# david-mathews-1994/deltarice

Hardware: AMD Instinct MI355X
Metric: encode+decode GB/s (int16 in) (higher is better)
Workload: dtype int16; 1 GPU; 1000000x7000 int16 Gaussian(sigma=10), m=8, 500 chunks of 2000x7000 per GPU, encode then decode, HBM resident; waveforms_per_gpu=1000000, wave_len=7000, rice_m=8, chunks_per_gpu=500, decode_impl=8

## Files before the change

### deltarice_amd/csrc/drx_encode.h

```cpp
#ifndef DRX_ENCODE_H
#define DRX_ENCODE_H
#include <hip/hip_runtime.h>
#include <stdint.h>

#include "drx_device.h"

namespace drx {

constexpr int kTile = 512;

typedef uint16_t u16x2 __attribute__((ext_vector_type(2)));
typedef int16_t i16x2 __attribute__((ext_vector_type(2)));
__device__ __forceinline__ u16x2 as_u16x2(uint32_t x) { return __builtin_bit_cast(u16x2, x); }
__device__ __forceinline__ i16x2 as_i16x2(uint32_t x) { return __builtin_bit_cast(i16x2, x); }
__device__ __forceinline__ uint32_t as_u32(u16x2 x) { return __builtin_bit_cast(uint32_t, x); }
__device__ __forceinline__ u16x2 splat(uint32_t v) { return (u16x2){(uint16_t)v, (uint16_t)v}; }

struct PackedCodes { uint32_t nb[4], c16[4], e[4]; };

template <bool GEN>
__device__ __forceinline__ void packed_codes(const uint32_t x[4], uint32_t xprev, uint32_t xprev2, const u16x2 (&tp)[4],
                                             uint32_t k, PackedCodes &c) {
    const u16x2 kv = splat(k), kp1 = splat(k + 1u), c16k = splat(16u - k);
    const u16x2 mlo = splat((1u << k) - 1u), mdelta = splat(0xffffu - ((1u << k) - 1u));
    u16x2 z[4], qc[4], e[4];
#pragma unroll
    for (int j = 0; j < 4; ++j) {
        const uint32_t xm1 = j ? x[j - 1] : xprev;
        const uint32_t before = __builtin_amdgcn_alignbit(x[j], xm1, 16);
        i16x2 d;
        if (GEN) {
            const uint32_t xm2 = j >= 2 ? x[j - 2] : (j == 1 ? xprev : xprev2);
            const uint32_t before3 = __builtin_amdgcn_alignbit(xm1, xm2, 16);
            d = __builtin_bit_cast(i16x2, (u16x2)(as_u16x2(x[j]) * tp[0] + as_u16x2(before) * tp[1] +
                                                  as_u16x2(xm1) * tp[2] + as_u16x2(before3) * tp[3]));
        } else {
            d = as_i16x2(x[j]) - as_i16x2(before);
        }
        z[j] = __builtin_bit_cast(u16x2, (i16x2)(d << (int16_t)1)) ^
               __builtin_bit_cast(u16x2, (i16x2)(d >> (int16_t)15));
    }
#pragma unroll
    for (int j = 0; j < 4; ++j) qc[j] = __builtin_elementwise_min((u16x2)(z[j] >> kv), splat(8u));
#pragma unroll
    for (int j = 0; j < 4; ++j) e[j] = qc[j] >> (uint16_t)3;
#pragma unroll
    for (int j = 0; j < 4; ++j) c.nb[j] = as_u32(e[j] * c16k + (qc[j] + kp1));
    const uint32_t mword = as_u32(splat(1u << k));
#pragma unroll
    for (int j = 0; j < 4; ++j) {
        const uint32_t mask = as_u32(e[j] * mdelta + mlo);
        c.c16[j] = (mask & as_u32(z[j])) | (~mask & mword);
        c.e[j] = as_u32(e[j]);
    }
}

constexpr uint32_t kEncCapWords = 2048;

__device__ __forceinline__ int load8_dwords(const int16_t *__restrict__ x, uint32_t len, uint32_t t0, int lane,
                                            bool vec_ok, uint32_t w[4]) {
    const uint32_t i0 = t0 + 8u * (uint32_t)lane;
    const int nv = (i0 >= len) ? 0 : (int)((len - i0) < 8u ? (len - i0) : 8u);
    if (vec_ok && nv == 8) {
        const uint4 q = *reinterpret_cast<const uint4 *>(x + i0);
        w[0] = q.x; w[1] = q.y; w[2] = q.z; w[3] = q.w;
    } else {
#pragma unroll
        for (int j = 0; j < 4; ++j) {
            const uint32_t a = (2 * j < nv) ? (uint32_t)(uint16_t)x[i0 + 2 * j] : 0u;
            const uint32_t b = (2 * j + 1 < nv) ? (uint32_t)(uint16_t)x[i0 + 2 * j + 1] : 0u;
            w[j] = a | (b << 16);
        }
    }
    return nv;
}

__device__ __forceinline__ void mask_tail(PackedCodes &c, int nv) {
#pragma unroll
    for (int j = 0; j < 4; ++j) {
        const uint32_t m = (2 * j + 1 < nv) ? 0xffffffffu : ((2 * j < nv) ? 0x0000ffffu : 0u);
        c.nb[j] &= m;
    }
}

__device__ __forceinline__ uint32_t lane_tile_bits(const PackedCodes &c) {
    const u16x2 s = as_u16x2(c.nb[0]) + as_u16x2(c.nb[1]) + as_u16x2(c.nb[2]) + as_u16x2(c.nb[3]);
    const uint32_t v = as_u32(s);
    return (v & 0xffffu) + (v >> 16);
}

template <bool FULL>
__device__ __forceinline__ void emit_tile(const PackedCodes &c, uint32_t pb) {
    typedef uint32_t __attribute__((address_space(3))) lds_u32;
#pragma unroll
    for (int j = 0; j < 8; ++j) {
        const uint32_t n = (j & 1) ? (c.nb[j >> 1] >> 16) : (c.nb[j >> 1] & 0xffffu);
        uint32_t code32 = __builtin_amdgcn_perm(c.e[j >> 1], c.c16[j >> 1], (j & 1) ? 0x07060302u : 0x05040100u);
        if (!FULL) code32 = n ? code32 : 0u;
        const uint32_t pe = pb + n;
        const uint64_t v = (uint64_t)code32 << (((pb & 32u) - pe) & 63u);
        lds_u32 *w = (lds_u32 *)(uintptr_t)((pb >> 3) & ~3u);
        __hip_atomic_fetch_or(w, (uint32_t)(v >> 32), __ATOMIC_RELAXED, __HIP_MEMORY_SCOPE_WORKGROUP);
        if ((uint32_t)v) __hip_atomic_fetch_or(w + 1, (uint32_t)v, __ATOMIC_RELAXED, __HIP_MEMORY_SCOPE_WORKGROUP);
        pb = pe;
    }
}

__device__ __forceinline__ void concat_codes(const PackedCodes &c, uint32_t (&w)[4]) {
    uint32_t w0 = 0, w1 = 0, w2 = 0, w3 = 0;
#pragma unroll
    for (int j = 0; j < 8; ++j) {
        const uint32_t nbj = c.nb[j >> 1];
        const uint32_t n = (j & 1) ? (nbj >> 16) : nbj;
        const uint32_t code32 = __builtin_amdgcn_perm(c.e[j >> 1], c.c16[j >> 1], (j & 1) ? 0x07060302u : 0x05040100u);
        const uint32_t s = 0u - n;
        if (j >= 3) w3 = __builtin_amdgcn_alignbit(w3, w2, s);
        if (j >= 2) w2 = __builtin_amdgcn_alignbit(w2, w1, s);
        if (j >= 1) w1 = __builtin_amdgcn_alignbit(w1, w0, s);
        w0 = (w0 << (n & 31u)) | code32;
    }
    w[0] = w0; w[1] = w1; w[2] = w2; w[3] = w3;
}

__device__ __forceinline__ void place_words(const uint32_t (&wd)[4], uint32_t pe) {
    typedef uint32_t __attribute__((address_space(3))) lds_u32;
    const uint32_t x0 = __builtin_amdgcn_alignbit(wd[0], 0u, pe);
    const uint32_t x1 = __builtin_amdgcn_alignbit(wd[1], wd[0], pe);
    const uint32_t x2 = __builtin_amdgcn_alignbit(wd[2], wd[1], pe);
    const uint32_t x3 = __builtin_amdgcn_alignbit(wd[3], wd[2], pe);
    const uint32_t x4 = __builtin_amdgcn_alignbit(0u, wd[3], pe);
    lds_u32 *w = (lds_u32 *)(uintptr_t)(((pe >> 3) & ~3u) - 16u);
    __hip_atomic_fetch_or(w + 4, x0, __ATOMIC_RELAXED, __HIP_MEMORY_SCOPE_WORKGROUP);
    __hip_atomic_fetch_or(w + 3, x1, __ATOMIC_RELAXED, __HIP_MEMORY_SCOPE_WORKGROUP);
    __hip_atomic_fetch_or(w + 2, x2, __ATOMIC_RELAXED, __HIP_MEMORY_SCOPE_WORKGROUP);
    if (x3 | x4) {
        __hip_atomic_fetch_or(w + 1, x3, __ATOMIC_RELAXED, __HIP_MEMORY_SCOPE_WORKGROUP);
        if (x4) __hip_atomic_fetch_or(w, x4, __ATOMIC_RELAXED, __HIP_MEMORY_SCOPE_WORKGROUP);
    }
}

constexpr uint32_t kBufFront = 4;

__device__ __forceinline__ void zero_row(uint32_t *row, uint32_t words, int lane) {
    for (int i = lane; i < (int)(words / 4u); i += 64) reinterpret_cast<uint4 *>(row)[i] = make_uint4(0, 0, 0, 0);
}

struct TileCodes {
    PackedCodes c;
    uint32_t cw[4], lane_bits, incl, tile_bits;
};

template <bool GEN, bool FULLT>
__device__ __forceinline__ TileCodes code_tile(const uint32_t (&w)[4], int nv, uint32_t &carry, uint32_t &carry2, const u16x2 (&tp)[4],
                                               uint32_t k) {
    TileCodes t;
    const uint32_t xprev = wave_shr1_carry(w[3], carry);
    carry = (uint32_t)__builtin_amdgcn_readlane((int)w[3], 63);
    uint32_t xprev2 = 0;
    if (GEN) {
        xprev2 = wave_shr1_carry(w[2], carry2);
        carry2 = (uint32_t)__builtin_amdgcn_readlane((int)w[2], 63);
    }
    packed_codes<GEN>(w, xprev, xprev2, tp, k, t.c);
    if (!FULLT) mask_tail(t.c, nv);
    t.lane_bits = lane_tile_bits(t.c);
    if (FULLT) concat_codes(t.c, t.cw);
    t.incl = wave_incl_scan_dpp(t.lane_bits);
    t.tile_bits = (uint32_t)__builtin_amdgcn_readlane((int)t.incl, 63);
    return t;
}

template <bool FULLT, typename At>
__device__ __forceinline__ void put_tile(const TileCodes &t, At &&at) {
    if (FULLT && !__any(t.lane_bits > 128u))
        place_words(t.cw, at(t.incl));
    else
        emit_tile<FULLT>(t.c, at(t.incl - t.lane_bits));
}

__device__ __forceinline__ void shr128(uint32_t (&w)[4], uint32_t n) {
    const uint32_t ws = n >> 5;
    const uint32_t y0 = ws == 0u ? w[0] : ws == 1u ? w[1] : ws == 2u ? w[2] : ws == 3u ? w[3] : 0u;
    const uint32_t y1 = ws == 0u ? w[1] : ws == 1u ? w[2] : ws == 2u ? w[3] : 0u;
    const uint32_t y2 = ws == 0u ? w[2] : ws == 1u ? w[3] : 0u;
    const uint32_t y3 = ws == 0u ? w[3] : 0u;
    w[0] = __builtin_amdgcn_alignbit(y1, y0, n);
    w[1] = __builtin_amdgcn_alignbit(y2, y1, n);
    w[2] = __builtin_amdgcn_alignbit(y3, y2, n);
    w[3] = y3 >> (n & 31u);
}

template <bool GEN>
__device__ __forceinline__ TileCodes code_tail_tile(const uint32_t (&w)[4], int nv, bool ragged, uint32_t &carry, uint32_t &carry2,
                                                    const u16x2 (&tp)[4], uint32_t k, bool &wide) {
    TileCodes t;
    const uint32_t xprev = wave_shr1_carry(w[3], carry);
    carry = (uint32_t)__builtin_amdgcn_readlane((int)w[3], 63);
    uint32_t xprev2 = 0;
    if (GEN) {
        xprev2 = wave_shr1_carry(w[2], carry2);
        carry2 = (uint32_t)__builtin_amdgcn_readlane((int)w[2], 63);
    }
    packed_codes<GEN>(w, xprev, xprev2, tp, k, t.c);
    const uint32_t all_bits = lane_tile_bits(t.c);
    concat_codes(t.c, t.cw);
    if (ragged) {
        PackedCodes cm = t.c;
        mask_tail(cm, nv);
        t.lane_bits = lane_tile_bits(cm);
        shr128(t.cw, all_bits - t.lane_bits);
    } else {
        t.lane_bits = nv ? all_bits : 0u;
#pragma unroll
        for (int j = 0; j < 4; ++j) t.cw[j] = nv ? t.cw[j] : 0u;
    }
    wide = __any((nv ? all_bits : 0u) > 128u);
    t.incl = wave_incl_scan_dpp(t.lane_bits);
    t.tile_bits = (uint32_t)__builtin_amdgcn_readlane((int)t.incl, 63);
    return t;
}

template <typename At>
__device__ __forceinline__ void put_tail_tile(const TileCodes &t, int nv, bool wide, At &&at) {
    if (!wide) {
        place_words(t.cw, at(t.incl));
    } else {
        PackedCodes c = t.c;
        mask_tail(c, nv);
        emit_tile<false>(c, at(t.incl - t.lane_bits));
    }
}

template <typename B, typename F>
__device__ __forceinline__ void for_full_tiles(const int16_t *__restrict__ x, uint32_t n_full, int lane, B &&between, F &&full) {
    constexpr int kDepth = 3;
    const uint4 *xv = reinterpret_cast<const uint4 *>(x) + lane;
    uint4 q[kDepth];
    uint32_t t = 0;
#pragma unroll
    for (int u = 0; u < kDepth; ++u) {
        q[u] = make_uint4(0, 0, 0, 0);
        if ((uint32_t)u < n_full) q[u] = xv[64 * (size_t)u];
    }
#pragma unroll 1
    for (; t + 2u * kDepth <= n_full; t += kDepth) {
        between();
#pragma unroll
        for (int u = 0; u < kDepth; ++u) {
            const uint32_t w[4] = {q[u].x, q[u].y, q[u].z, q[u].w};
            full(w);
            q[u] = xv[64 * (size_t)(t + u + kDepth)];
        }
    }
#pragma unroll 1
    for (; t < n_full; t += kDepth) {
        between();
#pragma unroll
        for (int u = 0; u < kDepth; ++u) {
            if (t + (uint32_t)u < n_full) {
                const uint32_t w[4] = {q[u].x, q[u].y, q[u].z, q[u].w};
                full(w);
                if (t + (uint32_t)u + kDepth < n_full) q[u] = xv[64 * (size_t)(t + u + kDepth)];
            }
        }
    }
}

template <typename B, typename F, typename T>
__device__ __forceinline__ void for_tiles(const int16_t *__restrict__ x, uint32_t len, uint32_t n_full, bool tail, int lane,
                                          B &&between, F &&full, T &&tailf) {
    constexpr int kDepth = 3;
    const uint32_t last = tail ? n_full : n_full - 1u;
    const uint32_t imax = len - 8u;
    auto load = [&](uint32_t tile) -> uint4 {
        tile = tile < last ? tile : last;
        uint32_t i = tile * (uint32_t)kTile + 8u * (uint32_t)lane;
        i = i < imax ? i : imax;
        return *reinterpret_cast<const uint4 *>(x + i);
    };
    uint4 q[kDepth];
#pragma unroll
    for (int u = 0; u < kDepth; ++u) {
        q[u] = load((uint32_t)u);
        __builtin_amdgcn_sched_barrier(0);
    }
    uint32_t t = 0;
#pragma unroll 1
    for (; t + kDepth <= n_full; t += kDepth) {
        between(true);
#pragma unroll
        for (int u = 0; u < kDepth; ++u) {
            const uint32_t w[4] = {q[u].x, q[u].y, q[u].z, q[u].w};
            full(w);
            q[u] = load(t + (uint32_t)u + kDepth);
        }
    }
    const uint32_t left = n_full - t;
    static_assert(kDepth == 3, "the straight code below");
    if (left) {
        between(false);
        const uint32_t w0[4] = {q[0].x, q[0].y, q[0].z, q[0].w};
        full(w0);
        if (left > 1u) {
            const uint32_t w1[4] = {q[1].x, q[1].y, q[1].z, q[1].w};
            full(w1);
        }
    }
    if (tail) {
        auto sel = [left](uint32_t a, uint32_t b, uint32_t c) -> uint32_t { return left == 0u ? a : (left == 1u ? b : c); };
        const uint32_t w[4] = {sel(q[0].x, q[1].x, q[2].x), sel(q[0].y, q[1].y, q[2].y), sel(q[0].z, q[1].z, q[2].z),
                               sel(q[0].w, q[1].w, q[2].w)};
        tailf(w);
    } else {
        __builtin_amdgcn_s_waitcnt(0x0f70);
    }
}

template <bool GEN, bool WINDOW>
__device__ __forceinline__ uint64_t recode_tiles(const int16_t *__restrict__ x, uint32_t len, uint32_t carry, uint32_t carry2,
                                                 const u16x2 (&tp)[4], uint32_t k, int lane, uint32_t *row, uint32_t row_words,
                                                 uint32_t *__restrict__ outp, uint32_t P0, uint32_t skip, uint32_t limit, uint64_t cap) {
    zero_row(row, row_words, lane);
    wave_sync();
    uint32_t *buf = row + kBufFront;
    const uint32_t buf_bits = lds_addr(buf) * 8u;
    auto mine = [&](uint64_t idx) -> bool { return !WINDOW || (idx >= skip && idx < limit && idx < cap); };
    uint64_t P = P0;
    uint32_t wn[4];
    int nvn = load8_dwords(x, len, 0u, lane, true, wn);
    for (uint32_t t0 = 0; t0 < len; t0 += kTile) {
        const uint32_t w[4] = {wn[0], wn[1], wn[2], wn[3]};
        const int nv = nvn;
        if (t0 + kTile < len) nvn = load8_dwords(x, len, t0 + kTile, lane, true, wn);
        const TileCodes t = code_tile<GEN, false>(w, nv, carry, carry2, tp, k);
        const uint64_t wfirst = P >> 5;
        const uint32_t at0 = buf_bits + (uint32_t)(P & 31u);
        put_tile<false>(t, [&](uint32_t bit) -> uint32_t { return at0 + bit; });
        P += t.tile_bits;
        wave_sync();
        const uint32_t nfull = (uint32_t)((P >> 5) - wfirst);
        for (uint32_t i = lane; i < nfull; i += 64) {
            if (mine(wfirst + i)) outp[wfirst + i] = buf[i];
            buf[i] = 0;
        }
        wave_sync();
        if (nfull && lane == 0) { const uint32_t cwd = buf[nfull]; buf[nfull] = 0; buf[0] = cwd; }
        wave_sync();
    }
    if (lane == 0) {
        if ((P & 31u) && mine(P >> 5)) outp[P >> 5] = buf[0];
        buf[0] = 0;
    }
    wave_sync();
    return P;
}

template <bool GEN>
__device__ __forceinline__ uint64_t recode_waveform(const int16_t *__restrict__ x, uint32_t len, const u16x2 (&tp)[4], uint32_t k, int lane,
                                                    uint32_t *row, uint32_t row_words, uint32_t *__restrict__ outp) {
    return recode_tiles<GEN, false>(x, len, 0u, 0u, tp, k, lane, row, row_words, outp, 0u, 0u, 0u, 0ull);
}

template <bool GEN>
__device__ __forceinline__ void history_before(const int16_t *__restrict__ x, uint32_t &carry, uint32_t &carry2) {
    carry = (uint32_t)(uint16_t)x[-1] << 16;
    if (GEN) {
        carry |= (uint32_t)(uint16_t)x[-2];
        carry2 = (uint32_t)(uint16_t)x[-4] | ((uint32_t)(uint16_t)x[-3] << 16);
    }
}

template <bool GEN>
__device__ __forceinline__ void recode_range(const int16_t *__restrict__ xw, uint32_t wf_len, uint32_t s_begin, uint32_t s_end, uint64_t Bp,
                                             uint32_t bits_mine, const u16x2 (&tp)[4], uint32_t k, int lane, uint32_t *row,
                                             uint32_t row_words, uint32_t *__restrict__ payload, uint64_t cap_words) {
    const uint32_t P0 = (uint32_t)(Bp & 31u);
    const uint64_t wbase = Bp >> 5;
    const uint32_t more = wf_len - s_end < 32u ? wf_len - s_end : 32u;
    uint32_t carry = 0, carry2 = 0;
    if (s_begin) history_before<GEN>(xw + s_begin, carry, carry2);
    recode_tiles<GEN, true>(xw + s_begin, s_end - s_begin + more, carry, carry2, tp, k, lane, row, row_words, payload + wbase, P0,
                            P0 ? 1u : 0u, (P0 + bits_mine + 31u) >> 5, cap_words > wbase ? cap_words - wbase : 0ull);
}

}
#endif
```

### deltarice_amd/csrc/drx_encode_stream.hip

```cpp
#include <hip/hip_runtime.h>
#include <stdint.h>

#include <type_traits>

#include "drx_internal.h"
#include "drx_device.h"
#include "drx_encode.h"

namespace drx {

constexpr int kEsWaves = 4;
constexpr uint32_t kEsFront = kBufFront;
constexpr uint32_t kEsBack = 12;
constexpr uint64_t kEsFlag = 1ull << 63;
constexpr uint32_t kEsCtrlWords = 32;
constexpr uint32_t kEsRing = kEsRingWords;
constexpr int kEsPollSleep = 4;

__device__ __forceinline__ uint64_t es_load(const uint64_t *p) {
    return __hip_atomic_load(p, __ATOMIC_RELAXED, __HIP_MEMORY_SCOPE_AGENT);
}
__device__ __forceinline__ void es_store(uint64_t *p, uint64_t v) {
    __hip_atomic_store(p, v, __ATOMIC_RELAXED, __HIP_MEMORY_SCOPE_AGENT);
}

constexpr uint32_t kScPer = 8;

__device__ __forceinline__ void es_scanner(uint64_t total, const uint64_t *__restrict__ size, uint64_t *__restrict__ place,
                                           DevStatus *st) {
    const int lane = lane_id();
    if (threadIdx.x >= 64) return;
    __builtin_amdgcn_s_setprio(3);
    uint64_t pos = 0, base = 0;
    uint32_t idle = 0;
    auto sample = [&](uint64_t (&v)[kScPer], uint64_t at) {
#pragma unroll
        for (int j = 0; j < (int)kScPer; ++j) {
            const uint64_t e = at + 64u * j + (uint32_t)lane;
            v[j] = e < total ? es_load(size + e) : kEsFlag;
        }
    };
    while (pos < total) {
        uint64_t v[kScPer];
        const uint64_t bs = pos;
        sample(v, pos);
        uint64_t run = 0;
        bool open = true, big = false;
#pragma unroll
        for (int j = 0; j < (int)kScPer; ++j) {
            const uint64_t e = bs + 64u * j + (uint32_t)lane;
            const uint64_t m = __ballot(e < pos || (v[j] >> 63) != 0);
            const uint32_t l = (m == ~0ull) ? 64u : (uint32_t)__builtin_ctzll(~m);
            run += open ? l : 0u;
            open = open && l == 64u;
            big = big || __any((v[j] & ~kEsFlag) >= (1ull << 24));
        }
        uint64_t end = bs + run;
        end = end < total ? end : total;
        if (end <= pos) {
            if (++idle > (1u << 22)) {
                if (lane == 0) atomicOr(&st->err, kErrInternal);
                return;
            }
            __builtin_amdgcn_s_sleep(1);
            continue;
        }
        idle = 0;
        uint64_t running = 0;
#pragma unroll
        for (int j = 0; j < (int)kScPer; ++j) {
            if (bs + 64u * j < end) {
                const uint64_t e = bs + 64u * j + (uint32_t)lane;
                const bool in = e >= pos && e < end;
                const uint64_t val = in ? (v[j] & ~kEsFlag) : 0ull;
                uint64_t inc;
                if (!big) {
                    inc = wave_incl_scan_dpp((uint32_t)val);
                } else {
                    inc = val;
#pragma unroll
                    for (int d = 1; d < 64; d <<= 1) {
                        const uint64_t t = __shfl_up(inc, d);
                        if (lane >= d) inc += t;
                    }
                }
                if (in) es_store(place + e, kEsFlag | (base + running + inc - val));
                running += big ? __shfl(inc, 63) : (uint64_t)(uint32_t)__builtin_amdgcn_readlane((int)(uint32_t)inc, 63);
            }
        }
        base += running;
        pos = end;
    }
}

template <int WV>
struct EsShared {
    uint32_t role, arrive, ticket[4];
    uint64_t mine[2][WV];
    uint32_t place_t[2];
};

template <int WV>
__device__ __forceinline__ uint32_t es_rendezvous(EsShared<WV> &shm, uint32_t cyc, int lane, int wv, uint32_t *__restrict__ ctrl,
                                                  uint64_t *__restrict__ size, uint32_t Tprev, uint64_t &off) {
    typedef uint32_t __attribute__((address_space(3))) lds_u32;
    uint32_t arr = 0;
    if (lane == 0) arr = __hip_atomic_fetch_add((lds_u32 *)&shm.arrive, 1u, __ATOMIC_RELAXED, __HIP_MEMORY_SCOPE_WORKGROUP);
    arr = (uint32_t)__builtin_amdgcn_readfirstlane((int)arr);
    if (arr == (uint32_t)WV * cyc) {
        if (lane == 0) shm.ticket[cyc & 3u] = atomicAdd(ctrl + 32, 1u);
    }
    __syncthreads();
    const uint32_t T = rfl(shm.ticket[cyc & 3u]);
    if (cyc) {
        uint64_t sum = 0, before = 0;
#pragma unroll
        for (int i = 0; i < WV; ++i) {
            const uint64_t m = rfl64(shm.mine[(cyc - 1u) & 1u][i]);
            sum += m;
            before += i < wv ? m : 0ull;
        }
        off = before;
        if (wv == 0 && lane == 0) es_store(size + Tprev, kEsFlag | sum);
    }
    return T;
}

template <uint32_t RING>
__device__ __forceinline__ uint32_t es_gap(bool pend, uint32_t startA, uint32_t start, uint32_t behind) {
    if (!pend) return RING - 8u;
    const uint32_t d = startA >= start ? startA - start : startA + RING - start;
    return d > behind ? d - behind : 0u;
}

template <typename InLds, typename Wait, typename Copy>
__device__ __forceinline__ bool es_release(bool must, uint64_t P, InLds &&place_in_lds, Wait &&wait_place, Copy &&copy_out) {
    decltype(wait_place()) pl;
    const bool seen = place_in_lds(pl);
    if (!(seen || must)) return false;
    if (!seen) __builtin_amdgcn_s_setprio(0);
    else if (P < (uint64_t)(4u * kTile * 7u)) __builtin_amdgcn_s_setprio(2);
    else __builtin_amdgcn_s_setprio(1);
    copy_out(seen ? pl : wait_place());
    return true;
}

template <uint32_t RING, typename Put>
__device__ __forceinline__ void ring_put_with(const TileCodes &t, uint32_t *row, uint32_t s0, int lane, Put &&put) {
    constexpr uint32_t kRingBits = RING * 32u;
    uint32_t *ring = row + kEsFront;
    const uint32_t ring_bits0 = lds_addr(ring) * 8u;
    put([&](uint32_t bit) -> uint32_t {
        const uint32_t b = s0 + bit;
        return ring_bits0 + (b >= kRingBits ? b - kRingBits : b);
    });
    if (s0 < kRingBits && s0 + t.tile_bits >= kRingBits) {
        wave_sync();
        if (lane < (int)kEsFront) {
            const uint32_t v = row[lane];
            if (v) { ring[RING - kEsFront + lane] |= v; row[lane] = 0; }
        } else if (lane < (int)(kEsFront + kEsBack)) {
            const uint32_t i = (uint32_t)lane - kEsFront, v = ring[RING + i];
            if (v) { ring[i] |= v; ring[RING + i] = 0; }
        }
        wave_sync();
    }
}
template <bool FULLT, uint32_t RING>
__device__ __forceinline__ void ring_put(const TileCodes &t, uint32_t *row, uint32_t s0, int lane) {
    ring_put_with<RING>(t, row, s0, lane, [&](auto &&at) { put_tile<FULLT>(t, at); });
}

static unsigned es_grid(const Geom &G, uint64_t tickets) {
    const unsigned full = 256u * (16u / kEsWaves);
    return (G.dbg & DRX_DBG_STREAM_THREE_WGS) ? 3u : (unsigned)(tickets + 1 < full ? tickets + 1 : full);
}

template <bool GEN, int WV, uint32_t RING>
__global__ __launch_bounds__(64 * WV, 4) void k_encode_stream(Geom G, const int16_t *__restrict__ in, uint32_t *__restrict__ out,
                                                              uint64_t out_cap, uint64_t *__restrict__ chunk_word_off,
                                                              uint32_t *__restrict__ wave_words, uint64_t *__restrict__ size,
                                                              uint64_t *__restrict__ place, uint32_t *__restrict__ ctrl,
                                                              DevStatus *st) {
    __shared__ __attribute__((aligned(16))) uint32_t ring_all[WV][kEsFront + RING + kEsBack];
    __shared__ EsShared<WV> shm;
    __shared__ uint64_t s_place_v[2];
    typedef uint32_t __attribute__((address_space(3))) lds_u32;
    typedef uint64_t __attribute__((address_space(3))) lds_u64;
    static_assert((kEsFront + RING + kEsBack) % 4 == 0 && RING % 4 == 0, "16-byte LDS accesses");
    constexpr uint32_t kRowWords = kEsFront + RING + kEsBack;
    const int lane = lane_id(), wv = wave_id();
    uint32_t *row = ring_all[wv];
    uint32_t *ring = row + kEsFront;

    if (threadIdx.x == 0) {
        shm.role = atomicAdd(ctrl, 1u);
        shm.arrive = 0;
        shm.place_t[0] = shm.place_t[1] = 0;
    }
    zero_row(row, kRowWords, lane);
    __syncthreads();
    const uint64_t n_tickets = (G.total_waves + WV - 1) / WV;
    if (rfl(shm.role) == 0) {
        es_scanner(n_tickets, size, place, st);
        return;
    }

    const uint32_t k = G.k;
    const u16x2 tp[4] = {splat(GEN ? G.enc_t[0] : 1u), splat(GEN ? G.enc_t[1] : 0xffffu), splat(GEN ? G.enc_t[2] : 0u),
                         splat(GEN ? G.enc_t[3] : 0u)};

    bool pend = false, fitsA = true;
    uint64_t gA = 0, offA = 0;
    uint32_t TA = 0, startA = 0, nA = 0;
    WaveRef rA = {};

    auto place_header = [&](const WaveRef &r, uint64_t g, uint32_t n, uint64_t ex, uint64_t &pos) -> bool {
        const uint64_t mine = 1ull + n + (r.idx == 0 ? 1ull : 0ull);
        pos = ex + (r.idx == 0 ? 1ull : 0ull);
        if (lane == 0) {
            if (r.idx == 0) chunk_word_off[r.chunk] = ex;
            if (g + 1 == G.total_waves) {
                chunk_word_off[G.n_chunks] = ex + mine;
                st->total_words = ex + mine;
                if (G.host_words) *G.host_words = ex + mine;
                if (ex + mine > out_cap) atomicOr(&st->err, kErrCapacity);
            }
        }
        const bool room = pos + 1u + n <= out_cap;
        if (room && lane == 0) {
            out[pos] = n;
            if (r.idx == 0) out[pos - 1] = r.n_samples;
        }
        return room;
    };
    auto copy_out = [&](uint64_t ex) {
        uint64_t pos;
        const bool room = place_header(rA, gA, nA, ex + offA, pos);
        uint32_t *__restrict__ outp = out + pos + 1;
        typedef uint32_t u32x4s __attribute__((ext_vector_type(4)));
        typedef u32x4s __attribute__((address_space(1), aligned(4))) g_u32x4_a4;
        const uint32_t n4 = nA & ~3u;
        for (uint32_t i = 4u * (uint32_t)lane; i < n4; i += 256u) {
            uint32_t w = startA + i;
            w = w >= RING ? w - RING : w;
            const uint4 v = *reinterpret_cast<const uint4 *>(ring + w);
            if (room) *(g_u32x4_a4 *)(outp + i) = (u32x4s){v.x, v.y, v.z, v.w};
            *reinterpret_cast<uint4 *>(ring + w) = make_uint4(0, 0, 0, 0);
        }
        if ((uint32_t)lane < nA - n4) {
            uint32_t w = startA + n4 + (uint32_t)lane;
            w = w >= RING ? w - RING : w;
            if (room) outp[n4 + (uint32_t)lane] = ring[w];
            ring[w] = 0;
        }
        wave_sync();
        pend = false;
    };
    auto place_in_lds = [&](uint64_t &ex) -> bool {
        const uint32_t t = __hip_atomic_load((lds_u32 *)&shm.place_t[TA & 1u], __ATOMIC_RELAXED, __HIP_MEMORY_SCOPE_WORKGROUP);
        if (rfl(t) != TA + 1u) return false;
        ex = rfl64(__hip_atomic_load((lds_u64 *)&s_place_v[TA & 1u], __ATOMIC_RELAXED, __HIP_MEMORY_SCOPE_WORKGROUP));
        return true;
    };
    auto place_to_lds = [&](uint64_t ex) {
        if (lane == 0) {
            __hip_atomic_store((lds_u64 *)&s_place_v[TA & 1u], ex, __ATOMIC_RELAXED, __HIP_MEMORY_SCOPE_WORKGROUP);
            __hip_atomic_store((lds_u32 *)&shm.place_t[TA & 1u], TA + 1u, __ATOMIC_RELAXED, __HIP_MEMORY_SCOPE_WORKGROUP);
        }
    };
    auto wait_place = [&]() -> uint64_t {
        uint32_t spins = 0;
        for (;;) {
            uint64_t ex;
            bool have = place_in_lds(ex);
            if (!have) {
                uint64_t v = 0;
                if (lane == 0) v = es_load(place + TA);
                const uint32_t hi = (uint32_t)__builtin_amdgcn_readfirstlane((int)(uint32_t)(v >> 32));
                if (hi >> 31) {
                    ex = ((uint64_t)(hi & 0x7fffffffu) << 32) | (uint32_t)__builtin_amdgcn_readfirstlane((int)(uint32_t)v);
                    place_to_lds(ex);
                    have = true;
                }
            }
            if (have) return ex;
            __builtin_amdgcn_s_sleep(kEsPollSleep);
            if (++spins > (1u << 22)) {
                if (lane == 0) atomicOr(&st->err, kErrInternal);
                return out_cap;
            }
        }
    };

    auto stream_out = [&](uint64_t ex) {
        uint64_t pos;
        const bool room = place_header(rA, gA, nA, ex + offA, pos);
        recode_waveform<GEN>(in + rA.sample_off, room ? rA.len : 0u, tp, k, lane, row, kRowWords, out + pos + 1);
        pend = false;
    };

    uint32_t start = 0;
    uint32_t Tprev = 0;
    for (uint32_t cyc = 0;; ++cyc) {
        const uint32_t T = es_rendezvous(shm, cyc, lane, wv, ctrl, size, Tprev, offA);
        if (pend && !fitsA) stream_out(wait_place());
        if ((uint64_t)T * WV >= G.total_waves) break;
        Tprev = T;
        const uint64_t g = (uint64_t)T * WV + (uint32_t)wv;
        if (g >= G.total_waves) {
            if (lane == 0) shm.mine[cyc & 1u][wv] = 0;
            if (pend) copy_out(wait_place());
            continue;
        }

        const WaveRef r = locate_uniform(G, g);
        const int16_t *x = in + r.sample_off;
        const uint32_t wlen = r.len;
        const uint32_t n_full = wlen / kTile, rem = wlen - n_full * (uint32_t)kTile;
        const bool tail = rem != 0u, ragged = (rem & 7u) != 0u;
        const bool tail_lane = 8u * (uint32_t)lane + 8u <= rem;

        auto gap = [&]() -> uint32_t { return es_gap<RING>(pend, startA, start, 8u); };
        if (pend && gap() < 512u) copy_out(wait_place());
        uint32_t limit = gap();

        uint64_t P = 0;
        bool fits = true;
        uint32_t carry = 0;
        uint32_t carry2 = 0;
        auto process_tile = [&](const uint32_t (&w)[4], int nv, auto full_tag) {
            constexpr bool FULLT = decltype(full_tag)::value;
            bool wide = false;
            TileCodes t;
            if constexpr (FULLT) t = code_tile<GEN, true>(w, nv, carry, carry2, tp, k);
            else t = code_tail_tile<GEN>(w, nv, ragged, carry, carry2, tp, k, wide);
            const uint32_t need = ((uint32_t)P + t.tile_bits + 31u) >> 5;
            bool ok = fits && need < limit;
            if (pend && es_release(fits && !ok, P, place_in_lds, wait_place, copy_out)) {
                limit = gap();
                ok = fits && need < limit;
            }
            if (ok) {
                if constexpr (FULLT) ring_put<true, RING>(t, row, start * 32u + (uint32_t)P, lane);
                else ring_put_with<RING>(t, row, start * 32u + (uint32_t)P, lane, [&](auto &&at) { put_tail_tile(t, nv, wide, at); });
            } else {
                fits = false;
            }
            P += t.tile_bits;
        };
        uint64_t pollv = 0;
        bool polling = false;
        auto between = [&](bool again) {
            if (!pend) return;
            if (polling) {
                const uint32_t hi = (uint32_t)__builtin_amdgcn_readfirstlane((int)(uint32_t)(pollv >> 32));
                polling = false;
                if (hi >> 31) {
                    place_to_lds(((uint64_t)(hi & 0x7fffffffu) << 32) | (uint32_t)__builtin_amdgcn_readfirstlane((int)(uint32_t)pollv));
                    return;
                }
            }
            if (!again) return;
            if (lane == 0) pollv = es_load(place + TA);
            polling = true;
        };

        auto full_tile = [&](const uint32_t (&w)[4]) { process_tile(w, 8, std::true_type{}); };
        auto tail_tile = [&](const uint32_t (&wq)[4]) {
            const uint32_t i0 = 8u * (uint32_t)lane;
            const int nv = tail_lane ? 8 : (i0 < rem ? (int)(rem - i0) : 0);
            uint32_t w[4];
#pragma unroll
            for (int j = 0; j < 4; ++j) w[j] = tail_lane ? wq[j] : 0u;
            if (ragged && nv > 0 && nv < 8) {
                const int16_t *xl = x + (size_t)n_full * kTile + i0;
#pragma unroll
                for (int j = 0; j < 4; ++j) {
                    const uint32_t a = (2 * j < nv) ? (uint32_t)(uint16_t)xl[2 * j] : 0u;
                    const uint32_t b = (2 * j + 1 < nv) ? (uint32_t)(uint16_t)xl[2 * j + 1] : 0u;
                    w[j] = a | (b << 16);
                }
            }
            process_tile(w, nv, std::false_type{});
        };
        if (wlen >= 8u) {
            for_tiles(x, wlen, n_full, tail, lane, between, full_tile, tail_tile);
        } else {
            const uint32_t none[4] = {0u, 0u, 0u, 0u};
            tail_tile(none);
        }
        const uint32_t n = (uint32_t)((P + 31u) >> 5);
        wave_sync();
        if (lane == 0) {
            wave_words[g] = n;
            shm.mine[cyc & 1u][wv] = 1ull + n + (r.idx == 0 ? 1ull : 0ull);
        }
        if (pend) copy_out(wait_place());
        pend = true;
        fitsA = fits;
        gA = g;
        rA = r;
        TA = T;
        startA = start;
        nA = n;
        if (fits) {
            start += (n + 3u) & ~3u;
            start = start >= RING ? start - RING : start;
        }
    }
    if (pend) copy_out(wait_place());
}

struct EsPlace2 { uint64_t whdr, bits; };

__device__ __forceinline__ void es_scanner_segs(uint64_t total, uint32_t tpw, uint32_t waves_per_chunk, const uint64_t *__restrict__ size,
                                                uint64_t *__restrict__ place, DevStatus *st) {
    const int lane = lane_id();
    if (threadIdx.x >= 64) return;
    __builtin_amdgcn_s_setprio(3);
    uint64_t pos = 0;
    uint64_t whdr = 1;
    uint64_t bits_in = 0;
    uint32_t idle = 0;
    const double rcp_tpw = 1.0 / (double)tpw;
    while (pos < total) {
        uint64_t v[kScPer];
        const uint64_t bs = pos;
#pragma unroll
        for (int j = 0; j < (int)kScPer; ++j) {
            const uint64_t e = bs + 64u * j + (uint32_t)lane;
            v[j] = e < total ? es_load(size + e) : 0ull;
        }
        uint64_t run = 0;
        bool open = true;
#pragma unroll
        for (int j = 0; j < (int)kScPer; ++j) {
            const uint64_t m = __ballot((v[j] >> 63) != 0);
            const uint32_t l = (m == ~0ull) ? 64u : (uint32_t)__builtin_ctzll(~m);
            run += open ? l : 0u;
            open = open && l == 64u;
        }
        const uint64_t end = bs + run;
        if (end <= pos) {
            if (++idle > (1u << 22)) {
                if (lane == 0) atomicOr(&st->err, kErrInternal);
                return;
            }
            __builtin_amdgcn_s_sleep(1);
            continue;
        }
        idle = 0;
#pragma unroll
        for (int j = 0; j < (int)kScPer; ++j) {
            if (bs + 64u * j < end) {
                const uint64_t e = bs + 64u * j + (uint32_t)lane;
                const bool in = e < end;
                const uint32_t val = in ? (uint32_t)(v[j] & 0xffffffffull) : 0u;
                const uint32_t e32 = (uint32_t)e;
                uint32_t g = (uint32_t)((double)e32 * rcp_tpw);
                uint32_t jj = e32 - g * tpw;
                if ((int32_t)jj < 0) { g -= 1u; jj += tpw; }
                if (jj >= tpw) { g += 1u; jj -= tpw; }
                const bool closing = in && jj + 1u == tpw;
                const uint32_t inc = wave_incl_scan_dpp(val), ex = inc - val;
                const int f = lane - (int)jj;
                const uint32_t exf = (uint32_t)__shfl((int)ex, f < 0 ? 0 : f);
                const uint64_t before = f < 0 ? bits_in + ex : (uint64_t)(ex - exf);
                const uint64_t nw = closing ? (before + val + 31ull) >> 5 : 0ull;
                const uint64_t contrib = closing ? 1ull + nw + (((g + 1u) % waves_per_chunk == 0u) ? 1ull : 0ull) : 0ull;
                uint64_t cinc;
                if (!__any(contrib >= (1ull << 24))) {
                    cinc = wave_incl_scan_dpp((uint32_t)contrib);
                } else {
                    cinc = contrib;
#pragma unroll
                    for (int d = 1; d < 64; d <<= 1) {
                        const uint64_t t = __shfl_up(cinc, d);
                        if (lane >= d) cinc += t;
                    }
                }
                const uint64_t my_whdr = whdr + cinc - contrib;
                if (in) {
                    es_store(place + 2u * e, kEsFlag | my_whdr);
                    es_store(place + 2u * e + 1u, kEsFlag | before);
                }
                const uint64_t left = end - (bs + 64u * j);
                const int li = __builtin_amdgcn_readfirstlane(left >= 64u ? 63 : (int)left - 1);
                const uint64_t wn = my_whdr + contrib, bn = closing ? 0ull : before + val;
                whdr = ((uint64_t)(uint32_t)__builtin_amdgcn_readlane((int)(uint32_t)(wn >> 32), li) << 32) | (uint32_t)__builtin_amdgcn_readlane((int)(uint32_t)wn, li);
                bits_in = ((uint64_t)(uint32_t)__builtin_amdgcn_readlane((int)(uint32_t)(bn >> 32), li) << 32) | (uint32_t)__builtin_amdgcn_readlane((int)(uint32_t)bn, li);
            }
        }
        pos = end;
    }
}

template <bool GEN, int WV, uint32_t RING>
__global__ __launch_bounds__(64 * WV, 4) void k_encode_stream_segs(Geom G, uint32_t seg_len, uint32_t tpw, const int16_t *__restrict__ in,
                                                                   uint32_t *__restrict__ out, uint64_t out_cap,
                                                                   uint64_t *__restrict__ chunk_word_off, uint32_t *__restrict__ wave_words,
                                                                   uint64_t *__restrict__ size, uint64_t *__restrict__ place,
                                                                   uint32_t *__restrict__ ctrl, DevStatus *st) {
    __shared__ __attribute__((aligned(16))) uint32_t ring_all[WV][kEsFront + RING + kEsBack];
    __shared__ EsShared<WV> shm;
    __shared__ uint64_t s_place_v[2][2];
    __shared__ uint32_t s_first[2][WV];
    typedef uint32_t __attribute__((address_space(3))) lds_u32;
    typedef uint64_t __attribute__((address_space(3))) lds_u64;
    static_assert((kEsFront + RING + kEsBack) % 4 == 0 && RING % 4 == 0, "16-byte LDS accesses");
    static_assert(WV == (int)kEsSegWaves, "es_seg_shape() counts tickets of kEsSegWaves segments");
    constexpr uint32_t kRowWords = kEsFront + RING + kEsBack;
    const int lane = lane_id(), wv = wave_id();
    uint32_t *row = ring_all[wv];
    uint32_t *ring = row + kEsFront;

    if (threadIdx.x == 0) {
        shm.role = atomicAdd(ctrl, 1u);
        shm.arrive = 0;
        shm.place_t[0] = shm.place_t[1] = 0;
    }
    zero_row(row, kRowWords, lane);
    __syncthreads();
    const uint64_t n_tickets = G.total_waves * tpw;
    if (rfl(shm.role) == 0) {
        es_scanner_segs(n_tickets, tpw, G.u_n_waves, size, place, st);
        return;
    }
    const uint32_t k = G.k;
    const u16x2 tp[4] = {splat(GEN ? G.enc_t[0] : 1u), splat(GEN ? G.enc_t[1] : 0xffffu), splat(GEN ? G.enc_t[2] : 0u),
                         splat(GEN ? G.enc_t[3] : 0u)};

    bool pend = false, fitsA = true, lastA = false, sibA = false;
    uint64_t gA = 0, offA = 0;
    uint32_t TA = 0, startA = 0, nA = 0, bitsA = 0, sbeginA = 0, sendA = 0, parA = 0;
    WaveRef rA = {};

    auto headers = [&](const WaveRef &r, const EsPlace2 &pl, uint64_t B) {
        if (lane != 0) return;
        if (sbeginA == 0u && r.idx == 0u) {
            chunk_word_off[r.chunk] = pl.whdr - 1u;
            if (pl.whdr - 1u < out_cap) out[pl.whdr - 1u] = r.n_samples;
        }
        if (lastA) {
            const uint64_t n = (B + bitsA + 31ull) >> 5;
            wave_words[gA] = (uint32_t)n;
            if (pl.whdr < out_cap) out[pl.whdr] = (uint32_t)n;
            if (gA + 1u == G.total_waves) {
                const uint64_t tot = pl.whdr + 1ull + n;
                chunk_word_off[G.n_chunks] = tot;
                st->total_words = tot;
                if (G.host_words) *G.host_words = tot;
                if (tot > out_cap) atomicOr(&st->err, kErrCapacity);
            }
        }
    };
    auto copy_out = [&](const EsPlace2 &pl) {
        const uint64_t B = pl.bits + offA;
        headers(rA, pl, B);
        const uint64_t w0 = pl.whdr + 1ull + (B >> 5);
        const uint32_t s = (uint32_t)B & 31u;
        const uint32_t i_lo = s ? 1u : 0u, i_hi = (s + bitsA + 31u) >> 5;
        const uint32_t nA4 = (nA + 3u) & ~3u, top = nA4 > i_hi ? nA4 : ((i_hi + 3u) & ~3u);
        if (sibA) {
            if (lane == 0) {
                const uint32_t F = s_first[parA][wv + 1], sh = bitsA & 31u;
                uint32_t wi = startA + (bitsA >> 5);
                wi = wi >= RING ? wi - RING : wi;
                ring[wi] |= F >> sh;
                if (sh) {
                    wi = wi + 1u >= RING ? wi + 1u - RING : wi + 1u;
                    ring[wi] |= F << (32u - sh);
                }
            }
            wave_sync();
        }
        uint32_t *__restrict__ outp = out + w0;
        const uint64_t room = out_cap > w0 ? out_cap - w0 : 0ull;
        typedef uint32_t u32x4s __attribute__((ext_vector_type(4)));
        typedef u32x4s __attribute__((address_space(1), aligned(4))) g_u32x4_a4;
        uint32_t carryw = 0;
        for (uint32_t i0 = 0; i0 < top; i0 += 256u) {
            const uint32_t i = i0 + 4u * (uint32_t)lane;
            uint4 v = make_uint4(0, 0, 0, 0);
            uint32_t w = startA + i;
            w = w >= RING ? w - RING : w;
            const bool inr = i < nA4;
            if (inr) v = *reinterpret_cast<const uint4 *>(ring + w);
            uint32_t pw = (uint32_t)__builtin_amdgcn_update_dpp(0, (int)v.w, 0x138, 0xf, 0xf, false);
            if (lane == 0) pw = carryw;
            carryw = (uint32_t)__builtin_amdgcn_readlane((int)v.w, 63);
            const uint32_t o0 = __builtin_amdgcn_alignbit(pw, v.x, s), o1 = __builtin_amdgcn_alignbit(v.x, v.y, s);
            const uint32_t o2 = __builtin_amdgcn_alignbit(v.y, v.z, s), o3 = __builtin_amdgcn_alignbit(v.z, v.w, s);
            if (i >= i_lo && i + 4u <= i_hi && (uint64_t)i + 4u <= room) {
                *(g_u32x4_a4 *)(outp + i) = (u32x4s){o0, o1, o2, o3};
            } else {
                if (i >= i_lo && i < i_hi && (uint64_t)i < room) outp[i] = o0;
                if (i + 1u >= i_lo && i + 1u < i_hi && (uint64_t)i + 1u < room) outp[i + 1u] = o1;
                if (i + 2u >= i_lo && i + 2u < i_hi && (uint64_t)i + 2u < room) outp[i + 2u] = o2;
                if (i + 3u >= i_lo && i + 3u < i_hi && (uint64_t)i + 3u < room) outp[i + 3u] = o3;
            }
            if (inr) *reinterpret_cast<uint4 *>(ring + w) = make_uint4(0, 0, 0, 0);
        }
        wave_sync();
        pend = false;
    };
    auto place_in_lds = [&](EsPlace2 &pl) -> bool {
        const uint32_t t = __hip_atomic_load((lds_u32 *)&shm.place_t[TA & 1u], __ATOMIC_RELAXED, __HIP_MEMORY_SCOPE_WORKGROUP);
        if (rfl(t) != TA + 1u) return false;
        pl.whdr = rfl64(__hip_atomic_load((lds_u64 *)&s_place_v[TA & 1u][0], __ATOMIC_RELAXED, __HIP_MEMORY_SCOPE_WORKGROUP));
        pl.bits = rfl64(__hip_atomic_load((lds_u64 *)&s_place_v[TA & 1u][1], __ATOMIC_RELAXED, __HIP_MEMORY_SCOPE_WORKGROUP));
        return true;
    };
    auto place_to_lds = [&](const EsPlace2 &pl) {
        if (lane == 0) {
            __hip_atomic_store((lds_u64 *)&s_place_v[TA & 1u][0], pl.whdr, __ATOMIC_RELAXED, __HIP_MEMORY_SCOPE_WORKGROUP);
            __hip_atomic_store((lds_u64 *)&s_place_v[TA & 1u][1], pl.bits, __ATOMIC_RELAXED, __HIP_MEMORY_SCOPE_WORKGROUP);
            __hip_atomic_store((lds_u32 *)&shm.place_t[TA & 1u], TA + 1u, __ATOMIC_RELAXED, __HIP_MEMORY_SCOPE_WORKGROUP);
        }
    };
    auto place_of = [&](uint64_t pv, EsPlace2 &pl) -> bool {
        const uint32_t lo = (uint32_t)pv, hi = (uint32_t)(pv >> 32);
        const uint32_t h0 = (uint32_t)__builtin_amdgcn_readlane((int)hi, 0), h1 = (uint32_t)__builtin_amdgcn_readlane((int)hi, 1);
        if (!((h0 & h1) >> 31)) return false;
        pl.whdr = ((uint64_t)(h0 & 0x7fffffffu) << 32) | (uint32_t)__builtin_amdgcn_readlane((int)lo, 0);
        pl.bits = ((uint64_t)(h1 & 0x7fffffffu) << 32) | (uint32_t)__builtin_amdgcn_readlane((int)lo, 1);
        return true;
    };
    auto wait_place = [&]() -> EsPlace2 {
        uint32_t spins = 0;
        for (;;) {
            EsPlace2 pl;
            if (place_in_lds(pl)) return pl;
            uint64_t pv = 0;
            if (lane < 2) pv = es_load(place + 2ull * TA + (uint32_t)lane);
            if (place_of(pv, pl)) {
                place_to_lds(pl);
                return pl;
            }
            __builtin_amdgcn_s_sleep(kEsPollSleep);
            if (++spins > (1u << 22)) {
                if (lane == 0) atomicOr(&st->err, kErrInternal);
                pl.whdr = out_cap;
                pl.bits = 0;
                return pl;
            }
        }
    };

    auto stream_out = [&](const EsPlace2 &pl) {
        const uint64_t B = pl.bits + offA;
        headers(rA, pl, B);
        recode_range<GEN>(in + rA.sample_off, rA.len, sbeginA, sendA, B, bitsA, tp, k, lane, row, kRowWords, out + pl.whdr + 1ull,
                          out_cap > pl.whdr + 1ull ? out_cap - pl.whdr - 1ull : 0ull);
        pend = false;
    };

    uint32_t start = 0;
    uint32_t Tprev = 0;
    for (uint32_t cyc = 0;; ++cyc) {
        const uint32_t T = es_rendezvous(shm, cyc, lane, wv, ctrl, size, Tprev, offA);
        if (pend && !fitsA) stream_out(wait_place());
        if ((uint64_t)T >= n_tickets) break;
        Tprev = T;
        const uint32_t gw = T / tpw, tj = T - gw * tpw;
        const uint64_t g = gw;
        const WaveRef r = locate_uniform(G, g);
        const uint32_t wlen = r.len;
        const uint32_t sgi = tj * (uint32_t)WV + (uint32_t)wv;
        const uint64_t sb64 = (uint64_t)sgi * seg_len;
        if (sb64 >= wlen) {
            if (lane == 0) shm.mine[cyc & 1u][wv] = 0;
            if (pend) copy_out(wait_place());
            continue;
        }
        const uint32_t s_begin = (uint32_t)sb64;
        const uint32_t s_end = wlen - s_begin > seg_len ? s_begin + seg_len : wlen;
        const bool sib = wv + 1 < WV && seg_len >= 32u && wlen - s_end >= 32u;
        const uint32_t more = sib ? 0u : (wlen - s_end < 32u ? wlen - s_end : 32u);
        const uint32_t slen = s_end - s_begin;
        const uint32_t clen = slen + more;
        const int16_t *x = in + r.sample_off + s_begin;

        auto gap = [&]() -> uint32_t { return es_gap<RING>(pend, startA, start, 12u); };
        if (pend && gap() < 512u) copy_out(wait_place());
        uint32_t limit = gap();

        uint64_t P = 0;
        uint32_t seg_bits = 0;
        bool first = true;
        bool fits = true;
        uint32_t carry = 0, carry2 = 0;
        if (s_begin) history_before<GEN>(x, carry, carry2);
        auto process_tile = [&](const uint32_t (&w)[4], int nv, int mark, auto full_tag) {
            constexpr bool FULLT = decltype(full_tag)::value;
            const TileCodes t = code_tile<GEN, FULLT>(w, nv, carry, carry2, tp, k);
            if (!FULLT && mark >= 0) seg_bits = (uint32_t)P + (mark ? (uint32_t)__builtin_amdgcn_readlane((int)t.incl, mark - 1) : 0u);
            const uint32_t need = ((uint32_t)P + t.tile_bits + 31u) >> 5;
            bool ok = fits && need < limit;
            if (pend && es_release(fits && !ok, P, place_in_lds, wait_place, copy_out)) {
                limit = gap();
                ok = fits && need < limit;
            }
            if (ok)
                ring_put<FULLT, RING>(t, row, start * 32u + (uint32_t)P, lane);
            else
                fits = false;
            P += t.tile_bits;
            if (first) {
                first = false;
                wave_sync();
                if (lane == 0) s_first[cyc & 1u][wv] = ring[start];
            }
        };
        const uint32_t n_fast = more ? slen / kTile : clen / kTile;
        uint64_t pollv = 0;
        bool polling = false;
        auto between = [&]() {
            if (!pend) return;
            if (polling) {
                polling = false;
                EsPlace2 pl;
                if (place_of(pollv, pl)) {
                    place_to_lds(pl);
                    return;
                }
            }
            pollv = 0;
            if (lane < 2) pollv = es_load(place + 2ull * TA + (uint32_t)lane);
            polling = true;
        };
        for_full_tiles(x, n_fast, lane, between, [&](const uint32_t (&w)[4]) { process_tile(w, 8, -1, std::true_type{}); });
        for (uint32_t t0 = n_fast * kTile; t0 < clen; t0 += kTile) {
            uint32_t w[4];
            const int nv = load8_dwords(x, clen, t0, lane, true, w);
            const int mark = (more && slen >= t0 && slen < t0 + (uint32_t)kTile) ? (int)((slen - t0) >> 3) : -1;
            process_tile(w, nv, mark, std::false_type{});
        }
        if (!more) seg_bits = (uint32_t)P;
        const uint32_t n = (uint32_t)((P + (sib ? 63u : 31u)) >> 5);
        wave_sync();
        if (lane == 0) shm.mine[cyc & 1u][wv] = seg_bits;
        if (pend) copy_out(wait_place());
        pend = true;
        fitsA = fits;
        gA = g;
        rA = r;
        TA = T;
        startA = start;
        nA = fits ? n : 0u;
        bitsA = seg_bits;
        sbeginA = s_begin;
        sendA = s_end;
        lastA = s_end == wlen;
        sibA = sib;
        parA = cyc & 1u;
        if (fits) {
            start += (n + 3u) & ~3u;
            start = start >= RING ? start - RING : start;
        }
    }
    if (pend) copy_out(wait_place());
}

hipError_t launch_encode_stream(const EncodeCall &c, uint64_t *d_scan) {
    const Geom &G = *c.G;
    const EncOut &o = c.out;
    const hipStream_t s = c.s;
    if (G.total_waves == 0) return hipSuccess;
    const uint64_t W = G.total_waves;
    const uint64_t tickets = (W + kEsWaves - 1) / kEsWaves;
    mark(c.ev, 0, s);
    hipError_t e = hipMemsetAsync(d_scan, 0, (2 * tickets + kEsCtrlWords) * sizeof(uint64_t), s);
    if (e != hipSuccess) return e;
    mark(c.ev, 1, s);
    mark(c.ev, 2, s);
    uint64_t *size = d_scan, *place = d_scan + tickets;
    uint32_t *ctrl = reinterpret_cast<uint32_t *>(d_scan + 2 * tickets);
    const unsigned grid = es_grid(G, tickets);
    if (G.n_taps)
        k_encode_stream<true, kEsWaves, kEsRing><<<grid, 64 * kEsWaves, 0, s>>>(G, c.d_in, o.d_out, o.out_cap, o.d_chunk_word_off, o.d_wave_words,
                                                                              size, place, ctrl, c.d_status);
    else
        k_encode_stream<false, kEsWaves, kEsRing><<<grid, 64 * kEsWaves, 0, s>>>(G, c.d_in, o.d_out, o.out_cap, o.d_chunk_word_off, o.d_wave_words,
                                                                               size, place, ctrl, c.d_status);
    mark(c.ev, 3, s);
    return hipGetLastError();
}

hipError_t launch_encode_stream_segs(const EncodeCall &c, uint32_t seg_target, uint64_t *d_scan) {
    const Geom &G = *c.G;
    const EncOut &o = c.out;
    const hipStream_t s = c.s;
    if (G.total_waves == 0) return hipSuccess;
    const EsSegShape sh = es_seg_shape(G.u_wave_len, seg_target);
    const uint64_t tickets = G.total_waves * sh.tpw;
    mark(c.ev, 0, s);
    hipError_t e = hipMemsetAsync(d_scan, 0, (3 * tickets + kEsCtrlWords) * sizeof(uint64_t), s);
    if (e != hipSuccess) return e;
    mark(c.ev, 1, s);
    mark(c.ev, 2, s);
    uint64_t *size = d_scan, *place = d_scan + tickets;
    uint32_t *ctrl = reinterpret_cast<uint32_t *>(d_scan + 3 * tickets);
    const unsigned grid = es_grid(G, tickets);
    if (G.n_taps)
        k_encode_stream_segs<true, kEsWaves, kEsRing><<<grid, 64 * kEsWaves, 0, s>>>(G, sh.seg_len, sh.tpw, c.d_in, o.d_out, o.out_cap, o.d_chunk_word_off,
                                                                                   o.d_wave_words, size, place, ctrl, c.d_status);
    else
        k_encode_stream_segs<false, kEsWaves, kEsRing><<<grid, 64 * kEsWaves, 0, s>>>(G, sh.seg_len, sh.tpw, c.d_in, o.d_out, o.out_cap, o.d_chunk_word_off,
                                                                                    o.d_wave_words, size, place, ctrl, c.d_status);
    mark(c.ev, 3, s);
    return hipGetLastError();
}

}
```

Baseline: 1556 GB/s.

## Encode full tiles in pairs with one packed wave scan and shared ring placement

The streaming encoder now processes two full tiles at once. It packs both tiles' per-lane bit counts into the 16-bit halves of a single DPP inclusive scan, does one space check and release round per pair, and writes both tiles to the ring with a single fold check. The tile load pipeline depth goes from 3 to 4 so that two pairs stay in flight. This is meant to halve the scan, readlane and placement-sync overhead per tile. In exchange it uses more registers to hold the pair state and the extra buffered loads, and it recomputes the codes on the slow path when any lane exceeds 128 bits. Packing assumes each tile's total bits fit in 16 bits.

```diff
diff --git a/deltarice_amd/csrc/drx_encode.h b/deltarice_amd/csrc/drx_encode.h
--- a/deltarice_amd/csrc/drx_encode.h
+++ b/deltarice_amd/csrc/drx_encode.h
@@ -170,6 +170,56 @@
     return t;
 }
 
+struct PairTile {
+    uint32_t w[4], xprev, xprev2;
+    uint32_t cw[4], lane_bits, incl, tile_bits;
+};
+
+template <bool GEN>
+__device__ __forceinline__ void code_tile_pair(const uint32_t (&wa)[4], const uint32_t (&wb)[4], uint32_t &carry, uint32_t &carry2,
+                                               const u16x2 (&tp)[4], uint32_t k, PairTile &a, PairTile &b) {
+    a.xprev = wave_shr1_carry(wa[3], carry);
+    b.xprev = wave_shr1_carry(wb[3], (uint32_t)__builtin_amdgcn_readlane((int)wa[3], 63));
+    carry = (uint32_t)__builtin_amdgcn_readlane((int)wb[3], 63);
+    a.xprev2 = b.xprev2 = 0;
+    if (GEN) {
+        a.xprev2 = wave_shr1_carry(wa[2], carry2);
+        b.xprev2 = wave_shr1_carry(wb[2], (uint32_t)__builtin_amdgcn_readlane((int)wa[2], 63));
+        carry2 = (uint32_t)__builtin_amdgcn_readlane((int)wb[2], 63);
+    }
+#pragma unroll
+    for (int j = 0; j < 4; ++j) { a.w[j] = wa[j]; b.w[j] = wb[j]; }
+    {
+        PackedCodes c;
+        packed_codes<GEN>(wa, a.xprev, a.xprev2, tp, k, c);
+        a.lane_bits = lane_tile_bits(c);
+        concat_codes(c, a.cw);
+    }
+    {
+        PackedCodes c;
+        packed_codes<GEN>(wb, b.xprev, b.xprev2, tp, k, c);
+        b.lane_bits = lane_tile_bits(c);
+        concat_codes(c, b.cw);
+    }
+    const uint32_t incl = wave_incl_scan_dpp(a.lane_bits | (b.lane_bits << 16));
+    const uint32_t total = (uint32_t)__builtin_amdgcn_readlane((int)incl, 63);
+    a.incl = incl & 0xffffu;
+    b.incl = incl >> 16;
+    a.tile_bits = total & 0xffffu;
+    b.tile_bits = total >> 16;
+}
+
+template <bool GEN, typename At>
+__device__ __forceinline__ void put_pair_tile(const PairTile &t, const u16x2 (&tp)[4], uint32_t k, At &&at) {
+    if (!__any(t.lane_bits > 128u)) {
+        place_words(t.cw, at(t.incl));
+    } else {
+        PackedCodes c;
+        packed_codes<GEN>(t.w, t.xprev, t.xprev2, tp, k, c);
+        emit_tile<true>(c, at(t.incl - t.lane_bits));
+    }
+}
+
 template <bool FULLT, typename At>
 __device__ __forceinline__ void put_tile(const TileCodes &t, At &&at) {
     if (FULLT && !__any(t.lane_bits > 128u))
@@ -266,10 +316,10 @@
     }
 }
 
-template <typename B, typename F, typename T>
+template <typename B, typename P, typename F, typename T>
 __device__ __forceinline__ void for_tiles(const int16_t *__restrict__ x, uint32_t len, uint32_t n_full, bool tail, int lane,
-                                          B &&between, F &&full, T &&tailf) {
-    constexpr int kDepth = 3;
+                                          B &&between, P &&pair, F &&full, T &&tailf) {
+    constexpr int kDepth = 4;
     const uint32_t last = tail ? n_full : n_full - 1u;
     const uint32_t imax = len - 8u;
     auto load = [&](uint32_t tile) -> uint4 {
@@ -284,32 +334,45 @@
         q[u] = load((uint32_t)u);
         __builtin_amdgcn_sched_barrier(0);
     }
+    static_assert(kDepth == 4, "the straight code below");
     uint32_t t = 0;
+    uint32_t set = 0;
 #pragma unroll 1
-    for (; t + kDepth <= n_full; t += kDepth) {
+    for (; t + 2u <= n_full; t += kDepth) {
         between(true);
-#pragma unroll
-        for (int u = 0; u < kDepth; ++u) {
-            const uint32_t w[4] = {q[u].x, q[u].y, q[u].z, q[u].w};
-            full(w);
-            q[u] = load(t + (uint32_t)u + kDepth);
+        {
+            const uint32_t wa[4] = {q[0].x, q[0].y, q[0].z, q[0].w};
+            const uint32_t wb[4] = {q[1].x, q[1].y, q[1].z, q[1].w};
+            pair(wa, wb);
+            q[0] = load(t + 4u);
+            q[1] = load(t + 5u);
+        }
+        if (t + 4u > n_full) {
+            t += 2u;
+            set = 2;
+            break;
+        }
+        {
+            const uint32_t wa[4] = {q[2].x, q[2].y, q[2].z, q[2].w};
+            const uint32_t wb[4] = {q[3].x, q[3].y, q[3].z, q[3].w};
+            pair(wa, wb);
+            q[2] = load(t + 6u);
+            q[3] = load(t + 7u);
         }
     }
     const uint32_t left = n_full - t;
-    static_assert(kDepth == 3, "the straight code below");
     if (left) {
         between(false);
-        const uint32_t w0[4] = {q[0].x, q[0].y, q[0].z, q[0].w};
-        full(w0);
-        if (left > 1u) {
-            const uint32_t w1[4] = {q[1].x, q[1].y, q[1].z, q[1].w};
-            full(w1);
-        }
+        const uint32_t w[4] = {set ? q[2].x : q[0].x, set ? q[2].y : q[0].y, set ? q[2].z : q[0].z, set ? q[2].w : q[0].w};
+        full(w);
     }
     if (tail) {
-        auto sel = [left](uint32_t a, uint32_t b, uint32_t c) -> uint32_t { return left == 0u ? a : (left == 1u ? b : c); };
-        const uint32_t w[4] = {sel(q[0].x, q[1].x, q[2].x), sel(q[0].y, q[1].y, q[2].y), sel(q[0].z, q[1].z, q[2].z),
-                               sel(q[0].w, q[1].w, q[2].w)};
+        const uint32_t ts = set + left;
+        auto sel = [ts](uint32_t a, uint32_t b, uint32_t c, uint32_t d) -> uint32_t {
+            return ts == 0u ? a : (ts == 1u ? b : (ts == 2u ? c : d));
+        };
+        const uint32_t w[4] = {sel(q[0].x, q[1].x, q[2].x, q[3].x), sel(q[0].y, q[1].y, q[2].y, q[3].y),
+                               sel(q[0].z, q[1].z, q[2].z, q[3].z), sel(q[0].w, q[1].w, q[2].w, q[3].w)};
         tailf(w);
     } else {
         __builtin_amdgcn_s_waitcnt(0x0f70);
diff --git a/deltarice_amd/csrc/drx_encode_stream.hip b/deltarice_amd/csrc/drx_encode_stream.hip
--- a/deltarice_amd/csrc/drx_encode_stream.hip
+++ b/deltarice_amd/csrc/drx_encode_stream.hip
@@ -145,6 +145,20 @@
     return true;
 }
 
+template <uint32_t RING>
+__device__ __forceinline__ void ring_fold(uint32_t *row, int lane) {
+    uint32_t *ring = row + kEsFront;
+    wave_sync();
+    if (lane < (int)kEsFront) {
+        const uint32_t v = row[lane];
+        if (v) { ring[RING - kEsFront + lane] |= v; row[lane] = 0; }
+    } else if (lane < (int)(kEsFront + kEsBack)) {
+        const uint32_t i = (uint32_t)lane - kEsFront, v = ring[RING + i];
+        if (v) { ring[i] |= v; ring[RING + i] = 0; }
+    }
+    wave_sync();
+}
+
 template <uint32_t RING, typename Put>
 __device__ __forceinline__ void ring_put_with(const TileCodes &t, uint32_t *row, uint32_t s0, int lane, Put &&put) {
     constexpr uint32_t kRingBits = RING * 32u;
@@ -154,23 +168,28 @@
         const uint32_t b = s0 + bit;
         return ring_bits0 + (b >= kRingBits ? b - kRingBits : b);
     });
-    if (s0 < kRingBits && s0 + t.tile_bits >= kRingBits) {
-        wave_sync();
-        if (lane < (int)kEsFront) {
-            const uint32_t v = row[lane];
-            if (v) { ring[RING - kEsFront + lane] |= v; row[lane] = 0; }
-        } else if (lane < (int)(kEsFront + kEsBack)) {
-            const uint32_t i = (uint32_t)lane - kEsFront, v = ring[RING + i];
-            if (v) { ring[i] |= v; ring[RING + i] = 0; }
-        }
-        wave_sync();
-    }
+    if (s0 < kRingBits && s0 + t.tile_bits >= kRingBits) ring_fold<RING>(row, lane);
 }
 template <bool FULLT, uint32_t RING>
 __device__ __forceinline__ void ring_put(const TileCodes &t, uint32_t *row, uint32_t s0, int lane) {
     ring_put_with<RING>(t, row, s0, lane, [&](auto &&at) { put_tile<FULLT>(t, at); });
 }
-
+template <bool GEN, uint32_t RING>
+__device__ __forceinline__ void ring_put_pair(const PairTile &a, const PairTile &b, const u16x2 (&tp)[4], uint32_t k, uint32_t *row,
+                                              uint32_t s0, int lane) {
+    constexpr uint32_t kRingBits = RING * 32u;
+    const uint32_t ring_bits0 = lds_addr(row + kEsFront) * 8u;
+    const uint32_t s1 = s0 + a.tile_bits;
+    put_pair_tile<GEN>(a, tp, k, [&](uint32_t bit) -> uint32_t {
+        const uint32_t p = s0 + bit;
+        return ring_bits0 + (p >= kRingBits ? p - kRingBits : p);
+    });
+    put_pair_tile<GEN>(b, tp, k, [&](uint32_t bit) -> uint32_t {
+        const uint32_t p = s1 + bit;
+        return ring_bits0 + (p >= kRingBits ? p - kRingBits : p);
+    });
+    if (s0 < kRingBits && s1 + b.tile_bits >= kRingBits) ring_fold<RING>(row, lane);
+}
 static unsigned es_grid(const Geom &G, uint64_t tickets) {
     const unsigned full = 256u * (16u / kEsWaves);
     return (G.dbg & DRX_DBG_STREAM_THREE_WGS) ? 3u : (unsigned)(tickets + 1 < full ? tickets + 1 : full);
@@ -349,6 +368,33 @@
             }
             P += t.tile_bits;
         };
+        auto process_pair = [&](const uint32_t (&wa)[4], const uint32_t (&wb)[4]) {
+            const uint32_t tagv = __hip_atomic_load((lds_u32 *)&shm.place_t[TA & 1u], __ATOMIC_RELAXED, __HIP_MEMORY_SCOPE_WORKGROUP);
+            __builtin_amdgcn_sched_barrier(0);
+            PairTile a, b;
+            code_tile_pair<GEN>(wa, wb, carry, carry2, tp, k, a, b);
+            const uint32_t bits = a.tile_bits + b.tile_bits;
+            const uint32_t need = ((uint32_t)P + bits + 31u) >> 5;
+            const uint32_t s0 = start * 32u + (uint32_t)P;
+            bool ok = false;
+#pragma unroll 1
+            for (int round = 0;; ++round) {
+                const bool must = round != 0;
+                auto look = [&](uint64_t &ex) -> bool {
+                    uint32_t tag = tagv;
+                    if (must) tag = __hip_atomic_load((lds_u32 *)&shm.place_t[TA & 1u], __ATOMIC_RELAXED, __HIP_MEMORY_SCOPE_WORKGROUP);
+                    if (rfl(tag) != TA + 1u) return false;
+                    ex = rfl64(__hip_atomic_load((lds_u64 *)&s_place_v[TA & 1u], __ATOMIC_RELAXED, __HIP_MEMORY_SCOPE_WORKGROUP));
+                    return true;
+                };
+                if (pend && es_release(must, P, look, wait_place, copy_out)) limit = gap();
+                ok = fits && need < limit;
+                if (ok || !fits || !pend || must) break;
+            }
+            if (ok) ring_put_pair<GEN, RING>(a, b, tp, k, row, s0, lane);
+            else fits = false;
+            P += bits;
+        };
         uint64_t pollv = 0;
         bool polling = false;
         auto between = [&](bool again) {
@@ -385,7 +431,7 @@
             process_tile(w, nv, std::false_type{});
         };
         if (wlen >= 8u) {
-            for_tiles(x, wlen, n_full, tail, lane, between, full_tile, tail_tile);
+            for_tiles(x, wlen, n_full, tail, lane, between, process_pair, full_tile, tail_tile);
         } else {
             const uint32_t none[4] = {0u, 0u, 0u, 0u};
             tail_tile(none);
```

Measured after the change: 1562 GB/s (median of 6 runs). No clear change (+0.4%).
